# MaciejKozarzewski/AlphaGomoku

Hardware: AMD Instinct MI355X
Metric: MCTS simulations/sec (self-play, 15x15 freestyle) (higher is better)
Workload: dtype f16 (network, fp32 accumulate) + int/fp32 (tree)

## Files before the change

### alphagomoku_amd/_lib.py

```python
import ctypes
import os

_HERE = os.path.dirname(os.path.abspath(__file__))
LIB_PATH = os.environ.get("AGX_LIB_PATH") or os.path.join(_HERE, "libagx.so")


class AgxError(RuntimeError):
    pass


class AgxNetDesc(ctypes.Structure):
    _fields_ = [("rows", ctypes.c_int), ("cols", ctypes.c_int), ("blocks", ctypes.c_int),
                ("filters", ctypes.c_int), ("in_channels", ctypes.c_int), ("value_hidden", ctypes.c_int),
                ("action_values", ctypes.c_int)]


_shared_torch_runtime = None


def share_torch_hip_runtime():
    global _shared_torch_runtime
    if _shared_torch_runtime is not None:
        return _shared_torch_runtime
    import importlib.util
# ... 227 lines not shown
    c.agx_engine_expand_backup_match.argtypes = [vp, vp]
    c.agx_engine_drain_records.argtypes = [vp, vp, ci, vp, ci, vp, vp]
    c.agx_engine_generate_openings.argtypes = [vp, vp, ci, ctypes.c_uint32, vp, vp]
    c.agx_engine_game_info.argtypes = [vp, ci, ctypes.POINTER(AgxGameInfo), vp, vp, ci]
    c.agx_engine_records.argtypes = [vp, vp, ci, vp, ci, ctypes.POINTER(ci), ctypes.POINTER(ci)]
    c.agx_engine_zobrist.argtypes = [vp, vp, sz]
    c.agx_engine_fetch_records.argtypes = [vp, vp, ci, vp, ci, vp, ci, vp, ci, ctypes.POINTER(AgxRecordCounts), ci]
    c.agx_game_buffer_create.argtypes = [ci, ci, ci, ci, ctypes.POINTER(vp)]
    c.agx_game_buffer_destroy.argtypes = [vp]
    c.agx_game_buffer_clear.argtypes = [vp]
    c.agx_game_buffer_collect.argtypes = [vp, vp, ctypes.POINTER(ci)]
    c.agx_game_buffer_stats.argtypes = [vp, ctypes.POINTER(AgxGameBufferStats)]
    c.agx_game_buffer_game.argtypes = [vp, ci, vp, sz, ctypes.POINTER(sz)]
    c.agx_game_buffer_save.argtypes = [vp, ctypes.c_char_p, ci]
    c.agx_game_buffer_load.argtypes = [vp, ctypes.c_char_p]
    c.agx_game_buffer_take_pending.argtypes = [vp, vp, ci, ci, vp, sz, ctypes.POINTER(sz)]
    c.agx_game_buffer_restore_pending.argtypes = [vp, vp, ci, ci, vp, sz]
    c.agx_game_buffer_forget_engine.argtypes = [vp, vp]
    c.agx_sample_v201_unpack.argtypes = [vp, sz, ci, ci, vp, vp, vp, vp, vp, vp, ctypes.POINTER(sz)]
    c.agx_debug_solve.argtypes = [vp, vp, vp, ci, vp, vp, vp, vp, vp, vp]
    c.agx_debug_new_generation.argtypes = [vp]
    c.agx_debug_solve_nodes.argtypes = [vp, ci, vp]
    c.agx_debug_pattern_state.argtypes = [vp, vp, vp, vp, ci, ci, vp, vp, vp, ci]
    c.agx_host_tables.argtypes = [ci, vp, vp, vp, vp]
    c.agx_make_opening.argtypes = [ci, ci, ctypes.c_uint32, vp]
    c.agx_get_outcome.argtypes = [ci, ci, vp, ci, ci, ci, ci, vp]


class AgxDatasetSample(ctypes.Structure):
    _fields_ = [(n, ctypes.c_int) for n in ["fragment", "game", "sample", "augmentation"]]


class AgxTensorShape(ctypes.Structure):
    _fields_ = [("rank", ctypes.c_int), ("dim", ctypes.c_int * 4)]


BATCH_INPUT_FP16, BATCH_POLICY_VISITS, BATCH_POLICY_VALUES = 1, 2, 4
BATCH_POLICY_FLAGS = {"torch_api": 0, "visits": BATCH_POLICY_VISITS, "values": BATCH_POLICY_VALUES}


class AgxBatchTensors(ctypes.Structure):
    _fields_ = [(n, ctypes.c_void_p) for n in ["input", "features", "policy", "value", "moves_left", "action_values", "action_values_weight"]]


def batch_policy_flag(policy):
    if policy not in BATCH_POLICY_FLAGS:
# ... 161 lines not shown
```

### alphagomoku_amd/csrc/dev_mcts.hpp

```cpp
#ifndef AGX_DEV_MCTS_HPP_
#define AGX_DEV_MCTS_HPP_

#include "dev_solver.hpp"
#include "root_noise.hpp"
#include "symmetry.hpp"

namespace agx
{
	namespace dev
	{
		__device__ __forceinline__ DNode* nodes_of(const EngineDev &E, int g, int arena) { return E.nodes + E.games[g].node_off[arena]; }
		__device__ __forceinline__ DEdge* edges_of(const EngineDev &E, int g, int arena) { return E.edges + E.games[g].edge_off[arena]; }
		__device__ __forceinline__ int* ht_of(const EngineDev &E, int g) { return E.ht + E.games[g].ht_off; }
		__device__ __forceinline__ void use_game_arenas(EngineDev &E, int g)
		{
			E.node_cap = E.games[g].node_cap;
			E.edge_cap = E.games[g].edge_cap;
			E.ht_cap = E.games[g].ht_cap;
		}

		__device__ inline int cache_seek(const EngineDev &E, const DNode *nodes, const int *ht, u64 hash, const u64 *cboard, int sign, int lane)
		{
			const int mask = E.ht_cap - 1;
			int slot = static_cast<int>(hash & static_cast<u64>(mask));
// ... 10 lines not shown
					same = (__ballot(!word_ok) == 0);
				}
				if (same)
					return idx - 1;
				slot = (slot + 1) & mask;
			}
			return -1;
		}
		__device__ __forceinline__ void node_head(DNode &dst, const DNode &src)
		{
			dst.edge_begin = src.edge_begin;
			dst.win = src.win;
			dst.draw = src.draw;
			dst.moves_left = src.moves_left;
			dst.visits = src.visits;
			dst.score = src.score;
			dst.n_edges = src.n_edges;
			dst.depth = src.depth;
			dst.vl = src.vl;
			dst.sign_to_move = src.sign_to_move;
			dst.flags = src.flags;
			dst.hash = src.hash;
		}
		__device__ inline int cache_seek_head(const EngineDev &E, const DNode *nodes, const int *ht, u64 hash, const u64 *cboard, int sign, int lane, DNode &head)
		{
			const int mask = E.ht_cap - 1;
			int slot = static_cast<int>(hash & static_cast<u64>(mask));
			for (int probes = 0; probes < E.ht_cap; probes++)
			{
				const int idx = ht[slot];
				if (idx == 0)
					return -1;
				const DNode &nd = nodes[idx - 1];
				DNode h;
				node_head(h, nd);
				const u64 word = (lane < BWORDS) ? nd.cboard[lane] : 0ull;
				bool same = (h.hash == hash) && (h.sign_to_move == sign);
				if (same)
				{
					const bool word_ok = (lane < BWORDS) ? (word == cboard[lane]) : true;
					same = (__ballot(!word_ok) == 0);
				}
				if (same)
				{
					head = h;
					return idx - 1;
				}
				slot = (slot + 1) & mask;
			}
			return -1;
		}
		__device__ inline void cache_insert(const EngineDev &E, int *ht, u64 hash, int node)
		{
// ... 17 lines not shown

		__device__ __forceinline__ unsigned long long symmetry_mix(unsigned long long z)
		{
			z += 0x9E3779B97F4A7C15ull;
			z = (z ^ (z >> 30)) * 0xBF58476D1CE4E5B9ull;
			z = (z ^ (z >> 27)) * 0x94D049BB133111EBull;
			return z ^ (z >> 31);
		}

		__device__ __forceinline__ void wave_argmax(float &value, int &index)
		{
			const uint32_t bits = __float_as_uint(value);
			const uint32_t key = (bits & 0x80000000u) ? ~bits : (bits | 0x80000000u);
			const uint32_t best = wave_reduce_umax(key);
			const uint32_t mine = (key == best) ? (0x7FFFFFFFu - static_cast<uint32_t>(index)) : 0u;
			index = static_cast<int>(0x7FFFFFFFu - wave_reduce_umax(mine));
			value = __uint_as_float((best & 0x80000000u) ? (best & 0x7FFFFFFFu) : ~best);
		}
		__device__ __forceinline__ uint32_t wave_max_u32(uint32_t v)
		{
			return wave_reduce_umax(v);
		}

		__device__ inline int select_edge(const EngineDev &E, const DNode &nd, const DEdge *edges, int lane, unsigned long long &edge_reads, const float *noisy_priors)
		{
			const int total = nd.visits + nd.vl;
			float c_puct = E.c_puct;
			if (E.c_scale != 0.0f)
				c_puct = static_cast<float>(static_cast<double>(E.c_puct) + static_cast<double>(E.c_scale) * det_log(static_cast<double>(total)));
			const float parent_sqrt_visit = static_cast<float>(static_cast<double>(c_puct) * sqrt(static_cast<double>(total)));
			float initial_q = 0.0f;
			if (E.init_to == 1)
				initial_q = nd.win + 0.5f * nd.draw;
			else if (E.init_to == 2)
				initial_q = 0.5f;

			float best_value = -3.402823466e+38f;
			int best = 0x7FFFFFFF;
			for (int i = lane; i < nd.n_edges; i += 64)
			{
				const DEdge e = edges[nd.edge_begin + i];
				float value;
				switch (s_pv(e.score))
				{
					case 0:
						value = -1000.0f + s_distance(e.score);
						break;
					case 1:
						value = 0.5f;
						break;
					case 3:
						value = +1000.0f - s_distance(e.score);
						break;
					default:
					{
						const int vl = e.flag_vl & 0x7FFF;
						const bool being_expanded = (e.flag_vl & 0x8000u) != 0;
						const float visits = 1.0e-8f + e.visits;
						const float virtual_loss = static_cast<float>(vl);
						const float vl_factor = visits / (visits + virtual_loss);
						const float expectation = e.win + 0.5f * e.draw;
						float Q;
						if (E.init_to == 0)
							Q = being_expanded ? -1000.0f : expectation * vl_factor;
						else
						{
							Q = initial_q;
							if (being_expanded)
								Q = -1000.0f;
							else if (e.visits > 0)
								Q = expectation * vl_factor;
						}
						const float prior = (noisy_priors != nullptr) ? noisy_priors[i] : e.prior;
						const float U = prior * parent_sqrt_visit / (1.0f + e.visits + vl);
						value = Q + U;
						break;
					}
				}
				if (value > best_value)
				{
					best_value = value;
					best = i;
				}
			}
			edge_reads += nd.n_edges;
			wave_argmax(best_value, best);
			return nd.edge_begin + best;
		}

		__device__ inline void correct_information_leak(DNode *nodes, DEdge *edges, const DTask &t, int path_len, int final_node, int lane)
		{
			float child_win = nodes[final_node].win, child_draw = nodes[final_node].draw;
			uint32_t child_score = nodes[final_node].score;
			for (int i = path_len - 1; i >= 0; i--)
			{
				const int node = t.path_node[i], e = t.path_edge[i];
				DNode nd;
				node_head(nd, nodes[node]);
				DEdge ed = edges[e];
				const float cw = ed.win, cd = ed.draw;
				const float tw = 1.0f - (child_win + child_draw), td = child_draw;
				const float scale = static_cast<float>(ed.visits) / static_cast<float>(nd.visits);
				const float nw = nd.win + (tw - cw) * scale, ndr = nd.draw + (td - cd) * scale;
				ed.win = tw;
				ed.draw = td;
				nd.win = nw;
				nd.draw = ndr;
				const uint32_t new_score = s_invert_up(child_score);
				ed.score = static_cast<uint16_t>(new_score);
				uint32_t result = 0;
// ... 41 lines not shown
```

### alphagomoku_amd/csrc/engine.hip

```cpp
#include "agx_internal.hpp"
#include "engine_types.hpp"
#include "dev_mcts.hpp"
#include "tables_host.hpp"
#include "renju_static.hpp"
#include "root_noise.hpp"
#include "sample_v201.hpp"

#include <vector>
#include <thread>
#include <chrono>
#include <mutex>
#include <cstring>
#include <algorithm>

using namespace agx;
using namespace agx::dev;

namespace
{
	__device__ __forceinline__ void select_batch(EngineDev &E, int tg, int g, int lane, uint8_t *sh_board, u64 *sh_cboard, const u64 *sh_keys)
	{
		GameState &gs = E.games[tg];
		GameState &ls = E.games[g];
		DNode *nodes = nodes_of(E, tg, gs.arena);
		DEdge *edges = edges_of(E, tg, gs.arena);
		const int *ht = ht_of(E, tg);
		const int n = E.n;

		int n_tasks = ls.n_tasks;
		int trials = 2 * E.batch_limit;
		unsigned long long st_levels = 0, st_edges = 0, st_leaks = 0, st_proven = 0, st_dup = 0;
		while (n_tasks < E.batch_limit)
		{
			const int root = gs.root;
			const int sims = (root < 0) ? 0 : nodes[root].visits;
			if (sims > E.max_sims)
				break;
			if (E.noise_type != 0 && root >= 0 && !gs.noise_ready && nodes[root].n_edges > 0)
			{
				if (lane == 0)
				{
					const DNode rn = nodes[root];
					const DEdge *root_edges = edges + rn.edge_begin;
					make_root_noise(E.noise_type, E.noise_weight, E.noise_seed, gs.opening_id, gs.n_moves, rn.n_edges, [&](int i) { return root_edges[i].prior; },
							E.noise + static_cast<size_t>(tg) * E.hw);
					gs.noise_ready = 1;
				}
				__threadfence_block();
				__syncthreads();
			}
			DTask &t = E.tasks[static_cast<size_t>(g) * E.batch + n_tasks];
			n_tasks++;
			for (int i = lane; i < E.hw; i += 64)
				sh_board[i] = gs.board[i];
			if (lane < BWORDS)
				sh_cboard[lane] = gs.cboard[lane];
			__syncthreads();
			int path_len = 0, final_node = -1, out = 0, sign = gs.sign_to_move;
			u64 hash = gs.root_hash;
			int last_edge = -1;
			int node = root;
			DNode nd;
			if (node >= 0)
				node_head(nd, nodes[node]);
			while (node >= 0)
			{
				if (path_len >= PATH_CAP)
				{
					if (lane == 0)
						ls.error = ERR_PATH_CAPACITY;
					break;
				}
				const int e = select_edge(E, nd, edges, lane, st_edges, (node == root && gs.noise_ready) ? E.noise + static_cast<size_t>(tg) * E.hw : nullptr);
				st_levels++;
				const DEdge ee = edges[e];
				const uint32_t mv = ee.move;
				const int s = mv & 3, cell = ((mv >> 2) & 127) * n + ((mv >> 9) & 127);
				const uint16_t flag_vl = static_cast<uint16_t>((ee.flag_vl & 0x8000u) | (((ee.flag_vl & 0x7FFF) + 1) & 0x7FFF));
				if (lane == 0)
				{
					sh_board[cell] = static_cast<uint8_t>(s);
					sh_cboard[cell >> 5] |= static_cast<u64>(s) << (2 * (cell & 31));
					t.path_node[path_len] = node;
					t.path_edge[path_len] = e;
					nodes[node].vl = static_cast<int16_t>(nd.vl + 1);
					edges[e].flag_vl = flag_vl;
				}
				hash ^= sh_keys[3 + 3 * cell] ^ sh_keys[3 + 3 * cell + s] ^ sh_keys[sign] ^ sh_keys[3 - s];
				sign = 3 - s;
				path_len++;
				last_edge = e;
				__syncthreads();
				if (s_proven(ee.score))
				{
					out = 2;
					break;
				}
				DNode child;
				node = cache_seek_head(E, nodes, ht, hash, sh_cboard, sign, lane, child);
				final_node = node;
				if (node < 0 && lane == 0)
					edges[e].flag_vl = static_cast<uint16_t>(flag_vl | 0x8000u);
				if (has_leak(E, ee, node >= 0, child.score, child.win, child.draw))
				{
					out = 1;
					break;
				}
				nd = child;
			}
			for (int i = lane; i < E.hw; i += 64)
				t.board[i] = sh_board[i];
			if (lane < BWORDS)
				t.cboard[lane] = sh_cboard[lane];
			if (lane == 0)
			{
				t.path_len = path_len;
				t.final_node = final_node;
				t.n_edges = 0;
				t.flags = t.flags & (TF_STATICALLY_SOLVED | TF_RECURSIVELY_SOLVED);
				t.sign_to_move = sign;
				t.score = s_unknown(0);
				t.win = 0.0f;
				t.draw = 0.0f;
				t.needs_nn = 0;
				t.hash = hash;
				if (out == 0 && path_len > gs.max_depth)
					gs.max_depth = path_len;
			}
			__syncthreads();
			if (path_len == 0)
				break;
			for (int i = 0; i < n_tasks - 1; i++)
			{
				const DTask &o = E.tasks[static_cast<size_t>(g) * E.batch + i];
				if (o.path_len > 0 && o.path_edge[o.path_len - 1] == last_edge)
				{
					st_dup++;
					break;
				}
			}
			if (out == 1)
			{
				correct_information_leak(nodes, edges, t, path_len, final_node, lane);
				cancel_virtual_loss(nodes, edges, t, path_len, lane);
				st_leaks++;
				n_tasks--;
			}
			if (out == 2 && lane == 0)
			{
				const uint32_t sc = edges[last_edge].score;
				float w, d;
				s_to_value(sc, w, d);
				t.final_node = -1;
				t.sign_to_move = 3 - sign;
				t.score = sc;
				t.win = w;
				t.draw = d;
				t.flags |= TF_BY_SOLVER | TF_SKIP_EDGE_GENERATION;
			}
			if (out == 2)
				st_proven++;
			__syncthreads();
			if (--trials <= 0)
				break;
		}
		if (lane == 0)
		{
			ls.n_tasks = n_tasks;
			ls.stats[2] += st_leaks;
			ls.stats[3] += st_proven;
			ls.stats[6] += st_levels;
			ls.stats[7] += st_edges;
			ls.stats[9] += st_dup;
		}
	}
	__global__ __launch_bounds__(64) void k_select(EngineDev E)
	{
		__shared__ uint8_t sh_board[MAXHW];
		__shared__ u64 sh_cboard[BWORDS];
		__shared__ u64 sh_keys[3 * (1 + MAXHW)];
		const int g = E.g0 + blockIdx.x, lane = threadIdx.x;
		const int tg = E.shared_tree ? 0 : g;
		GameState &gs = E.games[tg];
		if (!gs.active || gs.error != 0 || gs.outcome != 0 || gs.grow_pending)
			return;
		use_game_arenas(E, tg);
		for (int i = lane; i < 3 * (1 + E.hw); i += 64)
			sh_keys[i] = E.nc_keys[i];
		if (!E.shared_tree)
		{
			if (!gs.solve_pending)
				select_batch(E, g, g, lane, sh_board, sh_cboard, sh_keys);
			return;
		}
		for (int t = E.grp_first; t < E.grp_first + E.grp_count; t++)
		{
			if (E.games[t].error == 0)
// ... 1188 lines not shown
			{
				const int found = cache_seek(E, nodes, ht, t.hash, t.cboard, sign, lane);
				if (found < 0)
				{
					const int nid = gs.n_nodes, ebeg = gs.n_edges;
					if (nid >= E.node_cap || ebeg + n_e > E.edge_cap || 2 * (nid + 1) > E.ht_cap)
					{
						if (lane == 0)
							gs.error = (nid >= E.node_cap) ? ERR_NODE_CAPACITY : ((ebeg + n_e > E.edge_cap) ? ERR_EDGE_CAPACITY : ERR_HASH_TABLE);
						__syncthreads();
						return;
					}
					uint32_t max_score = 0;
					for (int i = lane; i < n_e; i += 64)
					{
						DEdge e;
						e.prior = e_prior[i];
						e.win = e_win[i];
						e.draw = e_draw[i];
						e.visits = 0;
						e.move = e_move[i];
						e.score = e_score[i];
						e.flag_vl = 0;
						e.pad = 0;
						edges[ebeg + i] = e;
						max_score = max(max_score, static_cast<uint32_t>(e_score[i]));
					}
					max_score = wave_max_u32(max_score);
					if (lane < BWORDS)
						nodes[nid].cboard[lane] = t.cboard[lane];
					if (lane == 0)
					{
						DNode &nd = nodes[nid];
						nd.edge_begin = ebeg;
						nd.n_edges = static_cast<int16_t>(n_e);
						nd.depth = static_cast<int16_t>(gs.n_moves + path_len);
						nd.vl = 0;
						nd.sign_to_move = static_cast<uint8_t>(sign);
						nd.pad8 = 0;
						nd.hash = t.hash;
						nd.visits = 1;
						const float tmp = static_cast<float>(1.0 / 1);
						float w = 0.0f + (win - 0.0f) * tmp, d = 0.0f + (draw - 0.0f) * tmp;
						nd.win = fmaxf(0.0f, fminf(1.0f, w));
						nd.draw = fmaxf(0.0f, fminf(1.0f, d));
						nd.moves_left = 0.0f + (moves_left - 0.0f) / 1;
						uint16_t nf = 0;
// ... 15 lines not shown
					final_node = nid;
					__syncthreads();
				}
				else
				{
					final_node = found;
					wasted++;
					if (path_len > 0)
					{
						const DEdge le = edges[t.path_edge[path_len - 1]];
						if (has_leak(E, le, true, nodes[found].score, nodes[found].win, nodes[found].draw))
							correct_information_leak(nodes, edges, t, path_len, final_node, lane);
					}
				}
			}

			if (lane == 0)
			{
				t.final_node = final_node;
				t.win = win;
				t.draw = draw;
				t.moves_left = moves_left;
				t.flags = flags;
			}
			__syncthreads();
		}

		for (int k = 0; k < n_tasks; k++)
		{
			DTask &t = E.tasks[static_cast<size_t>(g) * E.batch + k];
			const float win = t.win, draw = t.draw;
			const int path_len = t.path_len, sign = t.sign_to_move, final_node = t.final_node;
			float ml = t.moves_left;
			bool have_child = final_node >= 0;
			uint32_t child_score = have_child ? nodes[final_node].score : 0u;
#if AGX_WIDE_BACKUP
			if (path_len <= 64)
			{
				const bool mine = lane < path_len;
				const int node = mine ? t.path_node[lane] : 0, e = mine ? t.path_edge[lane] : 0;
				DNode nd;
				node_head(nd, nodes[node]);
				DEdge ed = edges[e];
				float ml_i = ml;
				for (int k = path_len - 1; k > lane; k--)
					ml_i += 1.0f;
// ... 298 lines not shown
			{
				const int ni = node_base + scan_nodes[tid] - 1, eb = edge_base + scan_edges[tid] - ne;
				DNode nd = nodes[i];
				cp_src = nd.edge_begin;
				cp_dst = eb;
				nd.edge_begin = eb;
				dst_nodes[ni] = nd;
				const int mask = E.ht_cap - 1;
				int slot = static_cast<int>(nd.hash & static_cast<u64>(mask));
				while (atomicCAS(&ht[slot], 0, ni + 1) != 0)
					slot = (slot + 1) & mask;
			}
			{
				const u64 *src64 = reinterpret_cast<const u64*>(edges);
				u64 *dst64 = reinterpret_cast<u64*>(dst_edges);
				for (int k = 0; k < 64; k++)
				{
					const int words = 3 * __builtin_amdgcn_readlane(ne, k);
					if (words == 0)
						continue;
					const size_t so = 3 * static_cast<size_t>(__builtin_amdgcn_readlane(cp_src, k)), dof = 3 * static_cast<size_t>(__builtin_amdgcn_readlane(cp_dst, k));
					for (int d = lane; d < words; d += 256)
					{
						const u64 w0 = src64[so + d];
						const u64 w1 = (d + 64 < words) ? src64[so + d + 64] : 0ull;
						const u64 w2 = (d + 128 < words) ? src64[so + d + 128] : 0ull;
						const u64 w3 = (d + 192 < words) ? src64[so + d + 192] : 0ull;
						dst64[dof + d] = w0;
						if (d + 64 < words)
							dst64[dof + d + 64] = w1;
						if (d + 128 < words)
							dst64[dof + d + 128] = w2;
						if (d + 192 < words)
							dst64[dof + d + 192] = w3;
					}
				}
			}
			node_base += scan_nodes[TPB - 1];
			edge_base += scan_edges[TPB - 1];
			__syncthreads();
		}
		u64 h = 0;
		for (int i = tid; i < E.hw; i += TPB)
			h ^= E.nc_keys[3 + 3 * i + gs.board[i]];
		block_reduce_xor<TPB>(h, scratch, tid);
		if (tid == 0)
		{
			gs.root_hash = h ^ E.nc_keys[gs.sign_to_move];
			gs.n_nodes = node_base;
			gs.n_edges = edge_base;
			gs.arena ^= 1;
			gs.generation = (gs.generation + 1) % 64;
			gs.max_depth = 0;
		}
		__syncthreads();
		if (wave == 0)
		{
// ... 256 lines not shown
				{
					eoff = -1;
					fits = false;
				}
			}
			if (E.record_format & 2)
			{
				soff = atomicAdd(&E.counters[6], (sbytes + 3) & ~3);
				if (soff + sbytes > E.sample_cap)
				{
					soff = -1;
					fits = false;
				}
			}
			sh_int[0] = (rec < E.record_cap) ? rec : -1;
			sh_int[1] = eoff;
			sh_int[6] = soff;
			sh_int[7] = fits ? 1 : 0;
		}
		__syncthreads();
		const int rec = sh_int[0], eoff = sh_int[1], soff = sh_int[6];
		if (eoff >= 0)
			for (int i = tid; i < root.n_edges; i += TPB)
				E.record_edges[eoff + i] = edges[root.edge_begin + i];
		if (soff >= 0)
		{
			const float prior_scale = v201::prior_scale(__uint_as_float(sh_max[0])), value_scale = v201::value_scale(__uint_as_float(sh_max[1]));
			const float visit_scale = v201::visit_scale(fmaxf(1.0f, static_cast<float>(sh_max[2])));
			uint8_t *out = E.samples + soff;
			if (tid == 0)
			{
				uint16_t *h16 = reinterpret_cast<uint16_t*>(out);
				h16[0] = static_cast<uint16_t>(v201::ScaleFormat::encode(value_scale));
				h16[1] = static_cast<uint16_t>(v201::ScaleFormat::encode(prior_scale));
				h16[2] = static_cast<uint16_t>(v201::ScaleFormat::encode(visit_scale));
				h16[3] = root.score;
				h16[4] = static_cast<uint16_t>(gs.n_moves);
				h16[5] = static_cast<uint16_t>((root.flags >> 3) & 7);
				*reinterpret_cast<uint32_t*>(out + 12) = static_cast<uint32_t>(n_entries);
			}
			for (int k = tid; k < n_entries; k += TPB)
			{
				const int cell = entry_cell[k], previous = (k > 0) ? entry_cell[k - 1] : 0;
				const int ei = (cell_edge[cell] & 0x7FFF) - 1;
				int visits = 0;
				float prior = 0.0f, win = 0.0f, draw = 0.0f;
				uint32_t score = s_unknown(0);
// ... 730 lines not shown
			for (int i = lane; i < nd.n_edges; i += 64)
			{
				const float value = best_edge_rating(edges[nd.edge_begin + i], nd);
				if (value > best_value)
				{
					best_value = value;
					best = i;
				}
			}
			wave_argmax(best_value, best);
			if (best >= nd.n_edges)
				break;
			const DEdge chosen = edges[nd.edge_begin + best];
			if (lane == 0)
			{
				out_pv[length] = chosen.move;
				query_write_edge(out_edges + length, chosen);
			}
			query_place(E, sh_cboard, q, chosen.move, lane);
			length++;
		}
		if (lane == 0)
			*out_length = length;
	}
	__global__ void k_reset_counter(int *counter, int *second)
	{
		*counter = 0;
		if (second != nullptr)
			*second = 0;
	}

	struct PositionJob
	{
			const uint8_t *boards;
			const uint8_t *signs;
			const int32_t *serials;
			int n, max_pv, max_steps;
			AgxPositionSearchOutputs out;
			AgxPositionSampleSink sink;
			int *cursor;
			int *finished;
			int *slot_position;
			int *slot_steps;
	};
	__device__ void position_write_empty(const PositionJob &J, int p, int hw, int status, int nodes, int edges, int steps, int error, int tid, int threads)
	{
// ... 1855 lines not shown
		return status;
	if (n_moves > 0)
		std::memcpy(e->query_host, h_moves, sizeof(uint16_t) * n_moves);
	AGX_HIP_CHECK(hipMemcpyAsync(e->query_dev, e->query_host, in_bytes, hipMemcpyHostToDevice, s));
	uint8_t *out_dev = e->query_dev + in_bytes, *out_host = e->query_host + in_bytes;
	const int tree = e->dev.shared_tree ? 0 : game;
	hipLaunchKernelGGL(k_principal_variation, dim3(1), dim3(64), 0, s, e->dev, tree, reinterpret_cast<const uint16_t*>(e->query_dev), n_moves, cap,
			reinterpret_cast<int*>(out_dev), reinterpret_cast<uint16_t*>(out_dev + len_bytes + node_bytes + edge_bytes),
			reinterpret_cast<AgxEdgeView*>(out_dev + len_bytes + node_bytes), reinterpret_cast<AgxNodeView*>(out_dev + len_bytes));
	AGX_HIP_CHECK(hipGetLastError());
	AGX_HIP_CHECK(hipMemcpyAsync(out_host, out_dev, out_bytes, hipMemcpyDeviceToHost, s));
	AGX_HIP_CHECK(hipStreamSynchronize(s));
	int n = 0;
	std::memcpy(&n, out_host, sizeof(int));
	*length = n;
	if (n > 0)
		std::memcpy(h_pv, out_host + len_bytes + node_bytes + edge_bytes, sizeof(uint16_t) * n);
	if (h_pv_edges != nullptr && n > 0)
		std::memcpy(h_pv_edges, out_host + len_bytes + node_bytes, sizeof(AgxEdgeView) * n);
	if (h_pv_nodes != nullptr)
		std::memcpy(h_pv_nodes, out_host + len_bytes, sizeof(AgxNodeView) * (n + 1));
	return AGX_OK;
}
int agx_engine_cancel_pending(AgxEngine *e, void *stream)
{
	AGX_REQUIRE(e != nullptr, AGX_ERR_INVALID, "agx_engine_cancel_pending: null engine");
	AGX_REQUIRE(e->begun, AGX_ERR_STATE, "agx_engine_cancel_pending: agx_engine_begin has not been called");
	AGX_REQUIRE(!e->dev.match_mode, AGX_ERR_STATE, "agx_engine_cancel_pending: a match-mode engine plays its own games");
	EngineDev d = e->dev;
	d.g0 = 0;
	hipLaunchKernelGGL(k_cancel_pending, dim3(d.shared_tree ? 1 : d.n_games), dim3(64), 0, static_cast<hipStream_t>(stream), d);
	AGX_HIP_CHECK(hipGetLastError());
	return AGX_OK;
}
int agx_engine_set_force_expand_root(AgxEngine *e, int force_expand_root)
{
	AGX_REQUIRE(e != nullptr, AGX_ERR_INVALID, "agx_engine_set_force_expand_root: null engine");
	AGX_REQUIRE(!e->dev.match_mode, AGX_ERR_STATE, "agx_engine_set_force_expand_root: a match-mode engine always prunes the root");
	e->dev.prune_root = force_expand_root ? 0 : 1;
	e->cfg.force_expand_root = force_expand_root ? 1 : 0;
	return AGX_OK;
}
int agx_engine_set_max_simulations(AgxEngine *e, int max_simulations)
{
	AGX_REQUIRE(e != nullptr && max_simulations > 0, AGX_ERR_INVALID, "agx_engine_set_max_simulations: invalid argument");
	e->dev.max_sims = max_simulations;
// ... 58 lines not shown
		FILE *f = fopen(getenv("AGX_SPEC_TRACE"), "w");
		if (f != nullptr)
		{
			for (size_t g = 0; g < games.size(); g++)
				fprintf(f, "%llu %llu %llu %llu\n", tr[4 * g], tr[4 * g + 1], tr[4 * g + 2], tr[4 * g + 3]);
			fclose(f);
		}
		std::vector<unsigned long long> wv(4 * static_cast<size_t>(std::max(e->spec_waves, 16)));
		AGX_HIP_CHECK(hipMemcpy(wv.data(), e->dev.spec_trace + 4 * games.size(), wv.size() * sizeof(unsigned long long), hipMemcpyDeviceToHost));
		f = fopen((std::string(getenv("AGX_SPEC_TRACE")) + ".waves").c_str(), "w");
		if (f != nullptr)
		{
			for (size_t w = 0; 4 * w < wv.size(); w++)
				fprintf(f, "%llu %llu %llu %llu\n", wv[4 * w], wv[4 * w + 1], wv[4 * w + 2], wv[4 * w + 3]);
			fclose(f);
		}
	}
	{
		unsigned long long p[16];
		AGX_HIP_CHECK(hipMemcpy(p, e->dev.spec_prof, sizeof(p), hipMemcpyDeviceToHost));
		fprintf(stderr, "[k_search_spec profile, wave-ms summed] select phase %.1f (slowest wave, max over launches %.3f ms), waiting for items %.1f, speculative solves %.1f (%llu, %.1f us each), "
				"commits + re-runs %.1f (longest %.3f ms), longest launch %.3f ms\n", p[0] / 1e5, p[1] / 1e5, p[2] / 1e5, p[3] / 1e5, p[6], p[3] / 1e2 / (p[6] ? p[6] : 1), p[4] / 1e5, p[5] / 1e5,
				p[7] / 1e5);
	}
#endif
#ifdef AGX_SOLVER_PROFILE
	{
		unsigned long long p[10] = { 0 };
		for (const GameState &g : games)
		{
			for (int i = 0; i < 6; i++)
				p[i] += g.prof[i];
			p[6] += g.prof[6] & 0xFFFFFFFFull;
			p[7] += g.prof[6] >> 32;
			p[8] += g.prof[7] & 0xFFFFFFFFull;
			p[9] += g.prof[7] >> 32;
		}
		fprintf(stderr, "[solver profile, 100 MHz ticks] solves %llu: set_board+encode %.1f us, frame machine %.1f us, place/remove %.1f us (%.1f per solve, %.2f us each), total %.1f us per solve\n",
				p[5], p[0] / 100.0 / p[5], p[1] / 100.0 / p[5], p[2] / 100.0 / p[5], (double) p[3] / p[5], p[2] / 100.0 / (p[3] ? p[3] : 1), p[4] / 100.0 / p[5]);
		fprintf(stderr, "[frame machine split, us per solve] table seek %.1f, move generation %.1f, ordering %.1f, evaluate+insert %.1f\n",
				p[6] / 100.0 / p[5], p[7] / 100.0 / p[5], p[8] / 100.0 / p[5], p[9] / 100.0 / p[5]);
		unsigned long long dp[24] = { 0 };
		for (const GameState &g : games)
			for (int i = 0; i < 24; i++)
				dp[i] += g.dprof[i];
		const double solves = static_cast<double>(p[5]);
// ... 56 lines not shown
		const DNode *nodes = e->dev.nodes + gs.node_off[gs.arena];
		AGX_HIP_CHECK(hipMemcpy(&root, nodes + gs.root, sizeof(DNode), hipMemcpyDeviceToHost));
		info->root_visits = root.visits;
		info->root_win = root.win;
		info->root_draw = root.draw;
		info->root_score = root.score;
		info->root_edges = root.n_edges;
		info->root_moves_left = root.moves_left;
		if (h_root_edges != nullptr)
		{
			AGX_REQUIRE(root.n_edges <= edge_capacity, AGX_ERR_INVALID, "agx_engine_game_info: %d root edges do not fit into %d", root.n_edges, edge_capacity);
			std::vector<DEdge> edges(root.n_edges);
			const DEdge *pool = e->dev.edges + gs.edge_off[gs.arena];
			AGX_HIP_CHECK(hipMemcpy(edges.data(), pool + root.edge_begin, edges.size() * sizeof(DEdge), hipMemcpyDeviceToHost));
			for (int i = 0; i < root.n_edges; i++)
			{
				h_root_edges[i].prior = edges[i].prior;
				h_root_edges[i].win = edges[i].win;
				h_root_edges[i].draw = edges[i].draw;
				h_root_edges[i].visits = edges[i].visits;
				h_root_edges[i].move = edges[i].move;
				h_root_edges[i].score = edges[i].score;
				h_root_edges[i].flag_and_virtual_loss = edges[i].flag_vl;
			}
		}
	}
	return AGX_OK;
}

int agx_engine_fetch_records(AgxEngine *e, AgxMoveRecord *h_records, int record_capacity, AgxEdgeView *h_edges, int edge_capacity, uint8_t *h_samples,
		int sample_capacity, AgxGameEnd *h_game_ends, int game_end_capacity, AgxRecordCounts *counts, int drain)
{
	AGX_REQUIRE(e != nullptr && counts != nullptr, AGX_ERR_INVALID, "agx_engine_fetch_records: null argument");
	AGX_HIP_CHECK(hipDeviceSynchronize());
	int counters[16];
	AGX_HIP_CHECK(hipMemcpy(counters, e->dev.counters, sizeof(counters), hipMemcpyDeviceToHost));
	const int nr = std::min(counters[3], e->dev.record_cap), ne = (e->dev.record_format & 1) ? std::min(counters[4], e->dev.record_edge_cap) : 0;
	const int ns = (e->dev.record_format & 2) ? std::min(counters[6], e->dev.sample_cap) : 0, ng = std::min(counters[7], e->dev.game_end_cap);
	counts->records = nr;
	counts->edges = ne;
	counts->sample_bytes = ns;
	counts->game_ends = ng;
	if (h_records != nullptr)
	{
		AGX_REQUIRE(nr <= record_capacity, AGX_ERR_INVALID, "agx_engine_fetch_records: %d records do not fit into %d", nr, record_capacity);
		std::vector<MoveRecordHeader> headers(nr);
// ... 1117 lines not shown
```

### alphagomoku_amd/csrc/engine_types.hpp

```cpp
#ifndef AGX_ENGINE_TYPES_HPP_
#define AGX_ENGINE_TYPES_HPP_

#include <cstdint>

namespace agx
{
	constexpr int MAXN = 20;
	constexpr int MAXHW = MAXN * MAXN;
	constexpr int BWORDS = 13;
	constexpr int PATH_CAP = 256;
	constexpr int SPEC_PARK_POOL = 128;
	constexpr int SPEC_PARK_WORDS = 2048 + 8;
	constexpr int MAX_FRAMES = 104;
	constexpr int OPENING_CAP = 32;

	struct alignas(16) FrameBytes { uint32_t w[8]; };

	struct DEdge
	{
			float prior;
			float win;
			float draw;
			int32_t visits;
			uint16_t move;
			uint16_t score;
			uint16_t flag_vl;
			uint16_t pad;
	};
	static_assert(sizeof(DEdge) == 24, "edge record must stay 24 bytes");

	struct DNode
	{
			int32_t edge_begin;
			float win;
			float draw;
			float moves_left;
			int32_t visits;
			uint16_t score;
			int16_t n_edges;
			int16_t depth;
			int16_t vl;
			uint8_t sign_to_move;
			uint8_t pad8;
			uint16_t flags;
			uint64_t hash;
			uint64_t cboard[BWORDS];
	};
	static_assert(sizeof(DNode) == 144, "node record layout");

	enum TaskFlags : uint32_t
	{
		TF_MUST_DEFEND = 1, TF_BY_NETWORK = 2, TF_BY_SOLVER = 4, TF_SKIP_EDGE_GENERATION = 8, TF_STATICALLY_SOLVED = 16, TF_RECURSIVELY_SOLVED = 32
// ... 29 lines not shown
			int32_t n_moves;
			int32_t outcome;
			int32_t root;
			int32_t n_nodes;
			int32_t n_edges;
			int32_t arena;
			int32_t n_tasks;
			int32_t need_move;
			int32_t generation;
			int32_t error;
			int32_t opening_id;
			int32_t games_done;
			int32_t solve_pos;
			int32_t solve_pending;
			int32_t nn_queued;
			int32_t noise_ready;
			int32_t my_sign;
			int32_t restart_id;
			int32_t match_score[4];
			int32_t arena_class;
			int32_t grow_pending;
			int32_t node_cap, edge_cap, ht_cap, grow_count;
			int32_t grow_owner, max_depth;
			uint64_t node_off[2], edge_off[2], ht_off;
			uint64_t new_node_off[2], new_edge_off[2], new_ht_off;
			uint64_t root_hash;
			uint64_t cboard[BWORDS];
			unsigned long long prof[8];
			unsigned long long dprof[24];
			unsigned long long spec_stats[4];
			unsigned long long stats[12];
			uint8_t board[MAXHW];
			uint16_t moves[MAXHW];
	};

	struct MoveRecordHeader
	{
			int32_t game_serial;
			int32_t move_number;
			uint16_t move;
			uint16_t root_score;
			int32_t root_visits;
			float root_win;
			float root_draw;
			int32_t n_edges;
			int32_t edge_offset;
// ... 142 lines not shown
```

### alphagomoku_amd/selfplay.py

```python
import ctypes

import numpy as np

from ._lib import (lib, check, AgxEngineConfig, AgxEngineBuffers, AgxEngineStats, AgxGameInfo, AgxEdgeView, AgxMoveRecord, AgxGameEnd, AgxSavedGame,
                   AgxRecordCounts, AgxGameBufferStats, AgxNodeView)

OPENING_CAP = 32


def default_config(**overrides):
    cfg = AgxEngineConfig()
    check(lib.agx_engine_default_config(ctypes.byref(cfg)))
    for k, v in overrides.items():
        if not hasattr(cfg, k):
            raise KeyError(k)
        setattr(cfg, k, v)
    return cfg


class HostPacer:

    def __init__(self, ahead=2):
        self.ahead = ahead
        self.count = 0
# ... 327 lines not shown
        counts = np.zeros(n, np.int32)
        flags = np.zeros(n, np.uint32)
        results = np.zeros(n, np.uint16)
        p = lambda a: a.ctypes.data_as(ctypes.c_void_p)
        check(lib.agx_debug_solve(self._h, p(boards), p(signs), n, p(feats), p(moves), p(scores), p(counts), p(flags), p(results)))
        nodes = np.zeros(n, np.uint64)
        check(lib.agx_debug_solve_nodes(self._h, n, p(nodes)))
        return dict(features=feats, moves=moves, scores=scores, counts=counts, flags=flags, results=results, nodes=nodes)

    def debug_pattern_state(self, boards, signs, moves):
        boards = np.ascontiguousarray(boards, dtype=np.uint8).reshape(-1, self.cells)
        signs = np.ascontiguousarray(signs, dtype=np.int32)
        moves = np.ascontiguousarray(moves, dtype=np.uint16)
        n = boards.shape[0]
        n_moves = moves.shape[1] if moves.size else 0
        stride = 2 * self.cells * 2 + 32
        pt = np.zeros((n, self.cells, 8), np.uint8)
        th = np.zeros((n, self.cells, 2), np.uint8)
        lists = np.zeros((n, stride), np.int16)
        p = lambda a: a.ctypes.data_as(ctypes.c_void_p)
        check(lib.agx_debug_pattern_state(self._h, p(boards), p(signs), p(moves), n, n_moves, p(pt), p(th), p(lists), stride))
        return pt, th, lists

    def close(self):
        if self._h:
            lib.agx_engine_destroy(self._h)
            self._h = ctypes.c_void_p()


def _edge_dict(e):
    return dict(move=e.move, visits=e.visits, prior=e.prior, win=e.win, draw=e.draw, score=e.score, flag_vl=e.flag_and_virtual_loss)


def _node_dict(v):
    return {name: getattr(v, name) for name, _ in v._fields_}


class GameBuffer:

    def __init__(self, rules, rows, cols, draw_after=0):
        self._h = ctypes.c_void_p()
        check(lib.agx_game_buffer_create(rules, rows, cols, draw_after, ctypes.byref(self._h)))

    def collect(self, pool):
        added = ctypes.c_int()
        check(lib.agx_game_buffer_collect(self._h, pool._h, ctypes.byref(added)))
# ... 33 lines not shown
```

### include/agx.h

```cpp
#ifndef AGX_H_
#define AGX_H_

#include <stddef.h>
#include <stdint.h>

#ifdef __cplusplus
extern "C" {
#endif

#define AGX_OK 0
#define AGX_ERR_INVALID 1
#define AGX_ERR_HIP 2
#define AGX_ERR_UNSUPPORTED 3
#define AGX_ERR_STATE 4

enum AgxRules { AGX_FREESTYLE = 0, AGX_STANDARD = 1, AGX_RENJU = 2, AGX_CARO5 = 3, AGX_CARO6 = 4 };

enum AgxSign { AGX_NONE = 0, AGX_CROSS = 1, AGX_CIRCLE = 2, AGX_ILLEGAL = 3 };

const char* agx_last_error(void);
int agx_version(void);
const char* agx_build_hash(void);
int agx_set_device(int device);
int agx_device_count(int* count);
// ... 242 lines not shown
	int n_edges;
} AgxNodeView;
int agx_engine_node_info(AgxEngine* engine, int game, const uint16_t* h_moves, const int* h_path_offsets, int n_paths,
		AgxNodeView* h_nodes, AgxEdgeView* h_edges, int edges_per_path, void* stream);
int agx_engine_principal_variation(AgxEngine* engine, int game, const uint16_t* h_moves, int n_moves, int max_length,
		uint16_t* h_pv, AgxEdgeView* h_pv_edges, AgxNodeView* h_pv_nodes, int* length, void* stream);
int agx_engine_records(AgxEngine* engine, AgxMoveRecord* h_records, int record_capacity, AgxEdgeView* h_edges, int edge_capacity, int* n_records, int* n_edges);
int agx_engine_drain_records(AgxEngine* engine, AgxMoveRecord* h_records, int record_capacity, AgxEdgeView* h_edges, int edge_capacity, int* n_records, int* n_edges);
int agx_engine_fetch_records(AgxEngine* engine, AgxMoveRecord* h_records, int record_capacity, AgxEdgeView* h_edges, int edge_capacity,
		uint8_t* h_samples, int sample_capacity, AgxGameEnd* h_game_ends, int game_end_capacity, AgxRecordCounts* counts, int drain);
int agx_engine_step_match(AgxEngine* engine, AgxNet* first_net, AgxNet* second_net, void* stream);
int agx_engine_select_solve_match(AgxEngine* engine, void* stream);
int agx_engine_expand_backup_match(AgxEngine* engine, void* stream);
int agx_engine_match_results(AgxEngine* engine, int* h_results, int pair_capacity);
int agx_engine_add_openings(AgxEngine* engine, const uint16_t* h_openings, int n_openings);
int agx_engine_zobrist(AgxEngine* engine, uint64_t* h_keys, size_t n_words);

int agx_debug_solve(AgxEngine* engine, const uint8_t* h_boards, const int* h_signs, int count, uint32_t* h_features, uint16_t* h_moves,
		uint16_t* h_scores, int* h_counts, uint32_t* h_flags, uint16_t* h_result_scores);
int agx_debug_solve_nodes(AgxEngine* engine, int count, unsigned long long* h_nodes);
int agx_debug_new_generation(AgxEngine* engine);
int agx_debug_pattern_state(AgxEngine* engine, const uint8_t* h_boards, const int* h_signs, const uint16_t* h_moves, int count, int n_moves,
		uint8_t* h_ptypes, uint8_t* h_threats, int16_t* h_lists, int lists_stride);
int agx_host_tables(int rules, uint8_t* h_pattern, uint8_t* h_half_open_three, uint8_t* h_threat, uint16_t* h_defense);

typedef struct AgxGameBuffer AgxGameBuffer;

typedef struct AgxGameBufferStats
{
	int games, samples, cross_win, draws, circle_win, game_length;
} AgxGameBufferStats;

int agx_game_buffer_create(int rules, int rows, int cols, int draw_after, AgxGameBuffer** out);
int agx_game_buffer_destroy(AgxGameBuffer* buffer);
int agx_game_buffer_clear(AgxGameBuffer* buffer);
int agx_game_buffer_collect(AgxGameBuffer* buffer, AgxEngine* engine, int* games_added);
int agx_game_buffer_stats(const AgxGameBuffer* buffer, AgxGameBufferStats* out);
int agx_game_buffer_game(const AgxGameBuffer* buffer, int index, uint8_t* h_bytes, size_t capacity, size_t* size);
int agx_game_buffer_save(const AgxGameBuffer* buffer, const char* path, int compress);
int agx_game_buffer_load(AgxGameBuffer* buffer, const char* path);
int agx_game_buffer_file_config(const char* path, int* rules, int* rows, int* cols);
int agx_game_buffer_take_pending(AgxGameBuffer* buffer, const AgxEngine* engine, int game_slot, int game_index, uint8_t* h_bytes, size_t capacity, size_t* size);
int agx_game_buffer_restore_pending(AgxGameBuffer* buffer, const AgxEngine* engine, int game_slot, int game_index, const uint8_t* h_bytes, size_t size);
int agx_game_buffer_forget_engine(AgxGameBuffer* buffer, const AgxEngine* engine);
int agx_game_buffer_config(const AgxGameBuffer* buffer, int* rules, int* rows, int* cols, int* draw_after);
int agx_sample_v201_unpack(const uint8_t* h_bytes, size_t size, int rows, int cols, int32_t* visits, float* prior, float* value, uint16_t* score,
// ... 248 lines not shown
```

Measured before the change: 1.039 million.

## Cache child node index in edge padding to skip hash-table probes during selection

Repurposes the edge record's pad field as a 16-bit child-node hint, written on expansion and after successful table lookups. Selection prefetches the hinted node while the virtual-loss stores happen, verifies it against hash, sign and board, and falls back to the hash probe on mismatch. The chosen edge is also taken from registers via readlane instead of re-read from memory, and the edge scan prefetches the next stride. Hints are masked out when edges are copied to a new arena or to records, and a debug kernel plus optional timing stamps are added. The cost is extra edge writes and the risk of stale hints, which are covered by the full position check.

New measurement: 1.038 million (median of 3 runs). About the same (-0.1%).

```diff
diff --git a/alphagomoku_amd/_lib.py b/alphagomoku_amd/_lib.py
--- a/alphagomoku_amd/_lib.py
+++ b/alphagomoku_amd/_lib.py
@@ -273,6 +273,7 @@
     c.agx_debug_new_generation.argtypes = [vp]
     c.agx_debug_solve_nodes.argtypes = [vp, ci, vp]
     c.agx_debug_pattern_state.argtypes = [vp, vp, vp, vp, ci, ci, vp, vp, vp, ci]
+    c.agx_debug_check_child_hints.argtypes = [vp, ci, vp]
     c.agx_host_tables.argtypes = [ci, vp, vp, vp, vp]
     c.agx_make_opening.argtypes = [ci, ci, ctypes.c_uint32, vp]
     c.agx_get_outcome.argtypes = [ci, ci, vp, ci, ci, ci, ci, vp]
diff --git a/alphagomoku_amd/csrc/dev_mcts.hpp b/alphagomoku_amd/csrc/dev_mcts.hpp
--- a/alphagomoku_amd/csrc/dev_mcts.hpp
+++ b/alphagomoku_amd/csrc/dev_mcts.hpp
@@ -56,13 +56,20 @@
 			dst.flags = src.flags;
 			dst.hash = src.hash;
 		}
-		__device__ inline int cache_seek_head(const EngineDev &E, const DNode *nodes, const int *ht, u64 hash, const u64 *cboard, int sign, int lane, DNode &head)
+		__device__ inline int cache_seek_head(const EngineDev &E, const DNode *nodes, const int *ht, u64 hash, const u64 *cboard, int sign, int lane, DNode &head,
+				unsigned long long *probe_ticks = nullptr)
 		{
 			const int mask = E.ht_cap - 1;
 			int slot = static_cast<int>(hash & static_cast<u64>(mask));
 			for (int probes = 0; probes < E.ht_cap; probes++)
 			{
+				const unsigned long long probe_begin = (probe_ticks != nullptr) ? wall_clock64() : 0ull;
 				const int idx = ht[slot];
+				if (probe_ticks != nullptr)
+				{
+					asm volatile("" :: "v"(idx));
+					*probe_ticks += wall_clock64() - probe_begin;
+				}
 				if (idx == 0)
 					return -1;
 				const DNode &nd = nodes[idx - 1];
@@ -126,7 +133,27 @@
 			return wave_reduce_umax(v);
 		}
 
-		__device__ inline int select_edge(const EngineDev &E, const DNode &nd, const DEdge *edges, int lane, unsigned long long &edge_reads, const float *noisy_priors)
+		__device__ __forceinline__ void node_request(const DNode *nodes, int candidate, int lane, DNode &head, u64 &word)
+		{
+			const DNode &nd = nodes[candidate];
+			node_head(head, nd);
+			word = (lane < BWORDS) ? nd.cboard[lane] : 0ull;
+		}
+		__device__ __forceinline__ bool node_is_position(const DNode &head, u64 word, u64 hash, const u64 *cboard, int sign, int lane)
+		{
+			const bool word_ok = (lane < BWORDS) ? (word == cboard[lane]) : true;
+			return (head.hash == hash) && (head.sign_to_move == sign) && (__ballot(!word_ok) == 0);
+		}
+
+		struct EdgeWords
+		{
+				uint32_t w[6];
+		};
+		static_assert(sizeof(EdgeWords) == sizeof(DEdge), "an edge record is six dwords");
+
+		template<bool KEEP>
+		__device__ inline int select_edge_impl(const EngineDev &E, const DNode &nd, const DEdge *edges, int lane, unsigned long long &edge_reads, const float *noisy_priors,
+				DEdge &chosen)
 		{
 			const int total = nd.visits + nd.vl;
 			float c_puct = E.c_puct;
@@ -141,9 +168,26 @@
 
 			float best_value = -3.402823466e+38f;
 			int best = 0x7FFFFFFF;
-			for (int i = lane; i < nd.n_edges; i += 64)
-			{
-				const DEdge e = edges[nd.edge_begin + i];
+			EdgeWords kept = { };
+			const int n_edges = nd.n_edges;
+			DEdge ahead = { };
+			float ahead_noisy = 0.0f;
+			if (lane < n_edges)
+			{
+				ahead = edges[nd.edge_begin + lane];
+				if (noisy_priors != nullptr)
+					ahead_noisy = noisy_priors[lane];
+			}
+			for (int i = lane; i < n_edges; i += 64)
+			{
+				const DEdge e = ahead;
+				const float noisy_prior = ahead_noisy;
+				if (i + 64 < n_edges)
+				{
+					ahead = edges[nd.edge_begin + i + 64];
+					if (noisy_priors != nullptr)
+						ahead_noisy = noisy_priors[i + 64];
+				}
 				float value;
 				switch (s_pv(e.score))
 				{
@@ -175,7 +219,7 @@
 							else if (e.visits > 0)
 								Q = expectation * vl_factor;
 						}
-						const float prior = (noisy_priors != nullptr) ? noisy_priors[i] : e.prior;
+						const float prior = (noisy_priors != nullptr) ? noisy_prior : e.prior;
 						const float U = prior * parent_sqrt_visit / (1.0f + e.visits + vl);
 						value = Q + U;
 						break;
@@ -185,11 +229,36 @@
 				{
 					best_value = value;
 					best = i;
-				}
-			}
-			edge_reads += nd.n_edges;
+					if constexpr (KEEP)
+						kept = __builtin_bit_cast(EdgeWords, e);
+				}
+			}
+			edge_reads += n_edges;
 			wave_argmax(best_value, best);
+			if constexpr (KEEP)
+			{
+				if (best < n_edges)
+				{
+					const int owner = __builtin_amdgcn_readfirstlane(best & 63);
+					EdgeWords w;
+#pragma unroll
+					for (int k = 0; k < 6; k++)
+						w.w[k] = static_cast<uint32_t>(__builtin_amdgcn_readlane(static_cast<int>(kept.w[k]), owner));
+					chosen = __builtin_bit_cast(DEdge, w);
+				}
+				else
+					chosen = edges[nd.edge_begin + best];
+			}
 			return nd.edge_begin + best;
+		}
+		__device__ inline int select_edge(const EngineDev &E, const DNode &nd, const DEdge *edges, int lane, unsigned long long &edge_reads, const float *noisy_priors)
+		{
+			DEdge unused;
+			return select_edge_impl<false>(E, nd, edges, lane, edge_reads, noisy_priors, unused);
+		}
+		__device__ inline int select_edge(const EngineDev &E, const DNode &nd, const DEdge *edges, int lane, unsigned long long &edge_reads, const float *noisy_priors, DEdge &chosen)
+		{
+			return select_edge_impl<true>(E, nd, edges, lane, edge_reads, noisy_priors, chosen);
 		}
 
 		__device__ inline void correct_information_leak(DNode *nodes, DEdge *edges, const DTask &t, int path_len, int final_node, int lane)
diff --git a/alphagomoku_amd/csrc/engine.hip b/alphagomoku_amd/csrc/engine.hip
--- a/alphagomoku_amd/csrc/engine.hip
+++ b/alphagomoku_amd/csrc/engine.hip
@@ -16,6 +16,31 @@
 using namespace agx;
 using namespace agx::dev;
 
+#ifndef AGX_SELECT_HINTS
+#define AGX_SELECT_HINTS 1
+#endif
+#if defined(AGX_SPEC_PROFILE) && defined(AGX_SELECT_STAMPS)
+#define SEL_STAMP_VARS() unsigned long long sel_t[8] = { 0, 0, 0, 0, 0, 0, 0, 0 }, sel_mark = 0, sel_probe = 0
+#define SEL_MARK() do { sel_mark = wall_clock64(); } while (0)
+#define SEL_WAIT(x) asm volatile("" :: "v"(x))
+#define SEL_LAP(k) do { const unsigned long long now_ = wall_clock64(); sel_t[k] += now_ - sel_mark; sel_mark = now_; } while (0)
+#define SEL_PROBE_BEGIN() do { sel_probe = 0; } while (0)
+#define SEL_PROBE_ARG &sel_probe
+#define SEL_PROBE_END(k_probe, k_rest) do { sel_t[k_probe] += sel_probe; sel_t[k_rest] -= sel_probe; } while (0)
+#define SEL_COUNT(k) do { sel_t[k]++; } while (0)
+#define SEL_FLUSH() do { if (lane == 0) for (int k_ = 0; k_ < 8; k_++) atomicAdd(&E.spec_prof[8 + k_], sel_t[k_]); } while (0)
+#else
+#define SEL_STAMP_VARS() do { } while (0)
+#define SEL_MARK() do { } while (0)
+#define SEL_WAIT(x) do { } while (0)
+#define SEL_LAP(k) do { } while (0)
+#define SEL_PROBE_BEGIN() do { } while (0)
+#define SEL_PROBE_ARG nullptr
+#define SEL_PROBE_END(k_probe, k_rest) do { } while (0)
+#define SEL_COUNT(k) do { } while (0)
+#define SEL_FLUSH() do { } while (0)
+#endif
+
 namespace
 {
 	__device__ __forceinline__ void select_batch(EngineDev &E, int tg, int g, int lane, uint8_t *sh_board, u64 *sh_cboard, const u64 *sh_keys)
@@ -26,10 +51,13 @@
 		DEdge *edges = edges_of(E, tg, gs.arena);
 		const int *ht = ht_of(E, tg);
 		const int n = E.n;
+		const int live_nodes = gs.n_nodes;
 
 		int n_tasks = ls.n_tasks;
 		int trials = 2 * E.batch_limit;
 		unsigned long long st_levels = 0, st_edges = 0, st_leaks = 0, st_proven = 0, st_dup = 0;
+		int st_hinted = 0;
+		SEL_STAMP_VARS();
 		while (n_tasks < E.batch_limit)
 		{
 			const int root = gs.root;
@@ -51,6 +79,8 @@
 			}
 			DTask &t = E.tasks[static_cast<size_t>(g) * E.batch + n_tasks];
 			n_tasks++;
+			SEL_MARK();
+			SEL_COUNT(7);
 			for (int i = lane; i < E.hw; i += 64)
 				sh_board[i] = gs.board[i];
 			if (lane < BWORDS)
@@ -62,7 +92,11 @@
 			int node = root;
 			DNode nd;
 			if (node >= 0)
+			{
 				node_head(nd, nodes[node]);
+				SEL_WAIT(static_cast<int>(nd.n_edges));
+			}
+			SEL_LAP(0);
 			while (node >= 0)
 			{
 				if (path_len >= PATH_CAP)
@@ -71,9 +105,22 @@
 						ls.error = ERR_PATH_CAPACITY;
 					break;
 				}
+				DEdge ee;
+#if AGX_SELECT_HINTS
+				const int e = select_edge(E, nd, edges, lane, st_edges, (node == root && gs.noise_ready) ? E.noise + static_cast<size_t>(tg) * E.hw : nullptr, ee);
+				SEL_LAP(1);
+				DNode hint_head;
+				u64 hint_word = 0;
+				const int hinted = child_hint_decode(ee.child_hint);
+				const bool try_hint = hinted >= 0 && hinted < live_nodes && !s_proven(ee.score);
+				if (try_hint)
+					node_request(nodes, hinted, lane, hint_head, hint_word);
+#else
 				const int e = select_edge(E, nd, edges, lane, st_edges, (node == root && gs.noise_ready) ? E.noise + static_cast<size_t>(tg) * E.hw : nullptr);
+				SEL_LAP(1);
+				ee = edges[e];
+#endif
 				st_levels++;
-				const DEdge ee = edges[e];
 				const uint32_t mv = ee.move;
 				const int s = mv & 3, cell = ((mv >> 2) & 127) * n + ((mv >> 9) & 127);
 				const uint16_t flag_vl = static_cast<uint16_t>((ee.flag_vl & 0x8000u) | (((ee.flag_vl & 0x7FFF) + 1) & 0x7FFF));
@@ -91,23 +138,47 @@
 				path_len++;
 				last_edge = e;
 				__syncthreads();
+				SEL_LAP(2);
 				if (s_proven(ee.score))
 				{
 					out = 2;
 					break;
 				}
 				DNode child;
-				node = cache_seek_head(E, nodes, ht, hash, sh_cboard, sign, lane, child);
+				SEL_PROBE_BEGIN();
+#if AGX_SELECT_HINTS
+				if (try_hint && node_is_position(hint_head, hint_word, hash, sh_cboard, sign, lane))
+				{
+					child = hint_head;
+					node = hinted;
+					st_hinted++;
+					SEL_COUNT(6);
+				}
+				else
+				{
+					node = cache_seek_head(E, nodes, ht, hash, sh_cboard, sign, lane, child, SEL_PROBE_ARG);
+					if (node >= 0 && lane == 0)
+						edges[e].child_hint = child_hint_encode(node);
+				}
+#else
+				node = cache_seek_head(E, nodes, ht, hash, sh_cboard, sign, lane, child, SEL_PROBE_ARG);
+#endif
 				final_node = node;
 				if (node < 0 && lane == 0)
 					edges[e].flag_vl = static_cast<uint16_t>(flag_vl | 0x8000u);
-				if (has_leak(E, ee, node >= 0, child.score, child.win, child.draw))
+				const bool leak = has_leak(E, ee, node >= 0, child.score, child.win, child.draw);
+				if (node >= 0)
+					SEL_WAIT(static_cast<int>(child.n_edges));
+				SEL_LAP(4);
+				SEL_PROBE_END(3, 4);
+				if (leak)
 				{
 					out = 1;
 					break;
 				}
 				nd = child;
 			}
+			SEL_MARK();
 			for (int i = lane; i < E.hw; i += 64)
 				t.board[i] = sh_board[i];
 			if (lane < BWORDS)
@@ -128,6 +199,7 @@
 					gs.max_depth = path_len;
 			}
 			__syncthreads();
+			SEL_LAP(5);
 			if (path_len == 0)
 				break;
 			for (int i = 0; i < n_tasks - 1; i++)
@@ -167,12 +239,14 @@
 		if (lane == 0)
 		{
 			ls.n_tasks = n_tasks;
+			ls.hint_levels = st_hinted;
 			ls.stats[2] += st_leaks;
 			ls.stats[3] += st_proven;
 			ls.stats[6] += st_levels;
 			ls.stats[7] += st_edges;
 			ls.stats[9] += st_dup;
 		}
+		SEL_FLUSH();
 	}
 	__global__ __launch_bounds__(64) void k_select(EngineDev E)
 	{
@@ -1407,7 +1481,7 @@
 						e.move = e_move[i];
 						e.score = e_score[i];
 						e.flag_vl = 0;
-						e.pad = 0;
+						e.child_hint = 0;
 						edges[ebeg + i] = e;
 						max_score = max(max_score, static_cast<uint32_t>(e_score[i]));
 					}
@@ -1469,6 +1543,8 @@
 				t.draw = draw;
 				t.moves_left = moves_left;
 				t.flags = flags;
+				if (n_e > 0 && path_len > 0)
+					edges[t.path_edge[path_len - 1]].child_hint = child_hint_encode(final_node);
 			}
 			__syncthreads();
 		}
@@ -1813,17 +1889,18 @@
 					const size_t so = 3 * static_cast<size_t>(__builtin_amdgcn_readlane(cp_src, k)), dof = 3 * static_cast<size_t>(__builtin_amdgcn_readlane(cp_dst, k));
 					for (int d = lane; d < words; d += 256)
 					{
+						const int r = d % 3;
 						const u64 w0 = src64[so + d];
 						const u64 w1 = (d + 64 < words) ? src64[so + d + 64] : 0ull;
 						const u64 w2 = (d + 128 < words) ? src64[so + d + 128] : 0ull;
 						const u64 w3 = (d + 192 < words) ? src64[so + d + 192] : 0ull;
-						dst64[dof + d] = w0;
+						dst64[dof + d] = (r == 2) ? (w0 & CHILD_HINT_WORD_MASK) : w0;
 						if (d + 64 < words)
-							dst64[dof + d + 64] = w1;
+							dst64[dof + d + 64] = (r == 1) ? (w1 & CHILD_HINT_WORD_MASK) : w1;
 						if (d + 128 < words)
-							dst64[dof + d + 128] = w2;
+							dst64[dof + d + 128] = (r == 0) ? (w2 & CHILD_HINT_WORD_MASK) : w2;
 						if (d + 192 < words)
-							dst64[dof + d + 192] = w3;
+							dst64[dof + d + 192] = (r == 2) ? (w3 & CHILD_HINT_WORD_MASK) : w3;
 					}
 				}
 			}
@@ -2126,7 +2203,11 @@
 		const int rec = sh_int[0], eoff = sh_int[1], soff = sh_int[6];
 		if (eoff >= 0)
 			for (int i = tid; i < root.n_edges; i += TPB)
-				E.record_edges[eoff + i] = edges[root.edge_begin + i];
+			{
+				DEdge snapshot = edges[root.edge_begin + i];
+				snapshot.child_hint = 0;
+				E.record_edges[eoff + i] = snapshot;
+			}
 		if (soff >= 0)
 		{
 			const float prior_scale = v201::prior_scale(__uint_as_float(sh_max[0])), value_scale = v201::value_scale(__uint_as_float(sh_max[1]));
@@ -2903,6 +2984,56 @@
 		}
 		if (lane == 0)
 			*out_length = length;
+	}
+	__global__ __launch_bounds__(64) void k_check_child_hints(EngineDev E, int t, int *out)
+	{
+		__shared__ u64 sh_cboard[BWORDS];
+		const int lane = threadIdx.x;
+		use_game_arenas(E, t);
+		const GameState &gs = E.games[t];
+		const DNode *nodes = nodes_of(E, t, gs.arena);
+		const DEdge *edges = edges_of(E, t, gs.arena);
+		const int *ht = ht_of(E, t);
+		const int n_nodes = gs.n_nodes;
+		int examined = 0, set = 0, wrong = 0;
+		for (int i = blockIdx.x; i < n_nodes; i += gridDim.x)
+		{
+			DNode nd;
+			node_head(nd, nodes[i]);
+			for (int k = 0; k < nd.n_edges; k++)
+			{
+				const DEdge ed = edges[nd.edge_begin + k];
+				const int s = ed.move & 3, cell = ((ed.move >> 2) & 127) * E.n + ((ed.move >> 9) & 127);
+				__syncthreads();
+				if (lane < BWORDS)
+					sh_cboard[lane] = nodes[i].cboard[lane] | ((lane == (cell >> 5)) ? (static_cast<u64>(s) << (2 * (cell & 31))) : 0ull);
+				__syncthreads();
+				const u64 hash = nd.hash ^ E.nc_keys[3 + 3 * cell] ^ E.nc_keys[3 + 3 * cell + s] ^ E.nc_keys[nd.sign_to_move] ^ E.nc_keys[3 - s];
+				const int child = cache_seek(E, nodes, ht, hash, sh_cboard, 3 - s, lane);
+				examined++;
+				if (ed.child_hint != 0)
+				{
+					set++;
+					const int hinted = child_hint_decode(ed.child_hint);
+					if (hinted >= n_nodes || hinted != child)
+						wrong++;
+				}
+			}
+		}
+		if (lane == 0)
+		{
+			atomicAdd(&out[0], examined);
+			atomicAdd(&out[1], set);
+			atomicAdd(&out[2], wrong);
+			if (blockIdx.x == 0)
+			{
+				int levels = gs.hint_levels;
+				if (E.shared_tree)
+					for (int r = 1; r < E.n_games; r++)
+						levels += E.games[r].hint_levels;
+				out[3] = levels;
+			}
+		}
 	}
 	__global__ void k_reset_counter(int *counter, int *second)
 	{
@@ -4804,6 +4935,21 @@
 		std::memcpy(h_pv_nodes, out_host + len_bytes, sizeof(AgxNodeView) * (n + 1));
 	return AGX_OK;
 }
+int agx_debug_check_child_hints(AgxEngine *e, int game, int *out4)
+{
+	AGX_REQUIRE(e != nullptr && out4 != nullptr, AGX_ERR_INVALID, "agx_debug_check_child_hints: null argument");
+	int status = query_tree(e, game, "agx_debug_check_child_hints");
+	if (status != AGX_OK)
+		return status;
+	AGX_HIP_CHECK(hipDeviceSynchronize());
+	if ((status = query_reserve(e, 4 * sizeof(int))) != AGX_OK)
+		return status;
+	AGX_HIP_CHECK(hipMemset(e->query_dev, 0, 4 * sizeof(int)));
+	hipLaunchKernelGGL(k_check_child_hints, dim3(64), dim3(64), 0, nullptr, e->dev, e->dev.shared_tree ? 0 : game, reinterpret_cast<int*>(e->query_dev));
+	AGX_HIP_CHECK(hipGetLastError());
+	AGX_HIP_CHECK(hipMemcpy(out4, e->query_dev, 4 * sizeof(int), hipMemcpyDeviceToHost));
+	return AGX_OK;
+}
 int agx_engine_cancel_pending(AgxEngine *e, void *stream)
 {
 	AGX_REQUIRE(e != nullptr, AGX_ERR_INVALID, "agx_engine_cancel_pending: null engine");
@@ -4908,6 +5054,15 @@
 		fprintf(stderr, "[k_search_spec profile, wave-ms summed] select phase %.1f (slowest wave, max over launches %.3f ms), waiting for items %.1f, speculative solves %.1f (%llu, %.1f us each), "
 				"commits + re-runs %.1f (longest %.3f ms), longest launch %.3f ms\n", p[0] / 1e5, p[1] / 1e5, p[2] / 1e5, p[3] / 1e5, p[6], p[3] / 1e2 / (p[6] ? p[6] : 1), p[4] / 1e5, p[5] / 1e5,
 				p[7] / 1e5);
+#ifdef AGX_SELECT_STAMPS
+		{
+			const unsigned long long levels = out->select_levels ? out->select_levels : 1, descents = p[15] ? p[15] : 1;
+			fprintf(stderr, "[select level stamps, hints %d] levels %llu (by hint %llu), descents %llu; per level, us: edge scan + argmax %.3f, chosen edge%s + virtual-loss stores + barrier %.3f, "
+					"table probe %.3f, child fetch + leak test %.3f; per descent, us: board copy + root head %.3f, task publish %.3f; wave-ms in all: levels %.1f, descents' overhead %.1f\n",
+					AGX_SELECT_HINTS, out->select_levels, p[14], p[15], p[9] / 1e2 / levels, AGX_SELECT_HINTS ? "" : " re-read", p[10] / 1e2 / levels, p[11] / 1e2 / levels, p[12] / 1e2 / levels,
+					p[8] / 1e2 / descents, p[13] / 1e2 / descents, (p[9] + p[10] + p[11] + p[12]) / 1e5, (p[8] + p[13]) / 1e5);
+		}
+#endif
 	}
 #endif
 #ifdef AGX_SOLVER_PROFILE
@@ -5010,6 +5165,7 @@
 				h_root_edges[i].move = edges[i].move;
 				h_root_edges[i].score = edges[i].score;
 				h_root_edges[i].flag_and_virtual_loss = edges[i].flag_vl;
+				h_root_edges[i].reserved = 0;
 			}
 		}
 	}
diff --git a/alphagomoku_amd/csrc/engine_types.hpp b/alphagomoku_amd/csrc/engine_types.hpp
--- a/alphagomoku_amd/csrc/engine_types.hpp
+++ b/alphagomoku_amd/csrc/engine_types.hpp
@@ -25,9 +25,17 @@
 			uint16_t move;
 			uint16_t score;
 			uint16_t flag_vl;
-			uint16_t pad;
+			uint16_t child_hint;
 	};
 	static_assert(sizeof(DEdge) == 24, "edge record must stay 24 bytes");
+
+	constexpr uint16_t child_hint_encode(int node) { return (node >= 0 && node < 0xFFFF) ? static_cast<uint16_t>(node + 1) : static_cast<uint16_t>(0); }
+	constexpr int child_hint_decode(uint16_t hint) { return static_cast<int>(hint) - 1; }
+	constexpr uint64_t CHILD_HINT_WORD_MASK = 0x0000FFFFFFFFFFFFull;
+	static_assert(child_hint_encode(-1) == 0 && child_hint_decode(0) == -1, "no node, no hint");
+	static_assert(child_hint_encode(0) == 1 && child_hint_decode(1) == 0, "node 0");
+	static_assert(child_hint_encode(65534) == 65535 && child_hint_decode(65535) == 65534, "the last node a hint can name");
+	static_assert(child_hint_encode(65535) == 0 && child_hint_encode(65536) == 0, "a node beyond 16 bits gets no hint");
 
 	struct DNode
 	{
@@ -103,6 +111,7 @@
 			int32_t grow_pending;
 			int32_t node_cap, edge_cap, ht_cap, grow_count;
 			int32_t grow_owner, max_depth;
+			int32_t hint_levels, hint_pad;
 			uint64_t node_off[2], edge_off[2], ht_off;
 			uint64_t new_node_off[2], new_edge_off[2], new_ht_off;
 			uint64_t root_hash;
diff --git a/alphagomoku_amd/selfplay.py b/alphagomoku_amd/selfplay.py
--- a/alphagomoku_amd/selfplay.py
+++ b/alphagomoku_amd/selfplay.py
@@ -373,6 +373,11 @@
         check(lib.agx_debug_pattern_state(self._h, p(boards), p(signs), p(moves), n, n_moves, p(pt), p(th), p(lists), stride))
         return pt, th, lists
 
+    def debug_check_child_hints(self, game=0):
+        out = np.zeros(4, np.int32)
+        check(lib.agx_debug_check_child_hints(self._h, int(game), out.ctypes.data_as(ctypes.c_void_p)))
+        return dict(edges=int(out[0]), hints_set=int(out[1]), hints_wrong=int(out[2]), levels_by_hint=int(out[3]))
+
     def close(self):
         if self._h:
             lib.agx_engine_destroy(self._h)
diff --git a/include/agx.h b/include/agx.h
--- a/include/agx.h
+++ b/include/agx.h
@@ -288,6 +288,7 @@
 int agx_debug_new_generation(AgxEngine* engine);
 int agx_debug_pattern_state(AgxEngine* engine, const uint8_t* h_boards, const int* h_signs, const uint16_t* h_moves, int count, int n_moves,
 		uint8_t* h_ptypes, uint8_t* h_threats, int16_t* h_lists, int lists_stride);
+int agx_debug_check_child_hints(AgxEngine* engine, int game, int* out);
 int agx_host_tables(int rules, uint8_t* h_pattern, uint8_t* h_half_open_three, uint8_t* h_threat, uint16_t* h_defense);
 
 typedef struct AgxGameBuffer AgxGameBuffer;
```
